# LucasAlegre/morl-baselines

Measured on NVIDIA B200. Metric: envelope_q_updates_per_sec, higher is better.
Workload: dtype f32

## Files before the change

### include/morl_b200.h

```cpp
#ifndef MORL_B200_H_
#define MORL_B200_H_

#include <stddef.h>
#include <stdint.h>

#ifdef __cplusplus
extern "C" {
#endif

#define MORL_B200_VERSION 100

#if defined(__GNUC__)
#define MORL_API __attribute__((visibility("default")))
#else
#define MORL_API
#endif

#define MORL_OK 0
#define MORL_ERR_NULL (-1)
#define MORL_ERR_SHAPE (-2)
#define MORL_ERR_ALIGN (-3)
#define MORL_ERR_UNSUPPORTED (-4)
#define MORL_ERR_NO_DEVICE (-5)

// ... 116 lines not shown
                                 float* q_out, void* stream);
MORL_API int morl_qhead_envelope_td_f32(int fmt, const void* a_on_planes, const void* a_tg_planes, long long a_plane_stride,
                                        const float* a_scale_on, const float* a_scale_tg, const void* w_on_planes, const void* w_tg_planes,
                                        long long w_plane_stride, const float* w_scale_on, const float* w_scale_tg, const float* bias_on,
                                        const float* bias_tg, int K, const float* wset, const float* reward, const float* done, float gamma,
                                        int B, int W, int A, int D, int dot_mode, int row_order, int reverse_tiles, float* target_out,
                                        int32_t* pref_out, int32_t* act_out, float* q_on_out, float* q_tg_out, void* stream);
MORL_API int morl_pairs_relu_split_planes(int fmt, const float* u, const float* v, int B, int W, int H, void* dst_planes,
                                          long long plane_stride, const float* scale, void* relu_bits_out, void* stream);


MORL_API size_t morl_gemm_mn_workspace_bytes(int M, int a_cols, int b_cols);
MORL_API int morl_gemm_planes_mn_f32(int fmt, const void* g_planes, long long g_plane_stride, int ldg, int g_cols, const float* g_scale,
                                     const void* h_planes, long long h_plane_stride, int ldh, int h_cols, const float* h_scale, int M,
                                     int transpose_out, float* out, int ld_out, float* colsum_out, void* workspace, void* stream);
MORL_API int morl_colsum_planes(int fmt, const void* planes, long long plane_stride, const float* scale, int M, int ld, int N, float* out,
                                void* workspace, void* stream);
MORL_API int morl_pairs_grad_reduce_planes(int fmt, const void* planes, long long plane_stride, const float* scale, int B, int W, int H,
                                           float* dU, float* dV, void* workspace, void* stream);

MORL_API int morl_pair_layer1_uv_f32(const float* feats, const float* wset, const float* W1, const float* b1, int B, int W, int F, int D, int H,
                                     float* u, float* v, void* stream);

MORL_API size_t morl_pair_layer1_grad_workspace_bytes(int F, int D, int H);
MORL_API int morl_pair_layer1_grad_f32(const float* dU, const float* dV, const float* feats, const float* wset, int B, int W, int F,
                              int D, int H, float* dW1, float* db1, void* workspace, void* stream);


MORL_API size_t morl_adam_workspace_bytes(int n_tensors, int64_t max_size);
MORL_API int morl_adam_clip_f32(float* const* params, const float* const* grads, float* const* exp_avg, float* const* exp_avg_sq,
// ... 8 lines not shown
```

### morl_baselines_b200/_lib.py

```python

from __future__ import annotations

import ctypes as C
import os

HERE = os.path.dirname(os.path.abspath(__file__))
LIB_PATH = os.path.join(HERE, "csrc", "libmorl_b200.so")

DOT_UNFUSED, DOT_FMA, DOT_PAIRFMA = 0, 1, 2
MAP_TILE, MAP_BLOCK = 0, 1
ROWS_REFERENCE, ROWS_BMAJOR = 0, 1
AC_ELEMENTWISE_MIN, AC_SCALAR_MIN, AC_ARGMIN_GATHER = 0, 1, 2
MAX_D = 8
FMT_BF16X3, FMT_F16X2 = 0, 1

_vp, _i, _f, _d, _i64, _sz = C.c_void_p, C.c_int, C.c_float, C.c_double, C.c_int64, C.c_size_t

SIGNATURES = {
    "morl_version": (_i, []),
    "morl_last_error": (C.c_char_p, []),
    "morl_device_sm_count": (_i, []),
    "morl_envelope_td_f32": (_i, [_vp, _vp, _vp, _vp, _vp, _f, _i, _i, _i, _i, _i, _i, _vp, _vp, _vp, _vp]),
    "morl_greedy_td_f32": (_i, [_vp, _vp, _vp, _i, _i, _vp, _vp, _i, _i, _f, _i, _i, _i, _i, _vp, _vp, _vp]),
    "morl_critic_min_td_f32": (_i, [_vp, _i, _vp, _i, _i, _vp, _vp, _i, _i, _f, _i, _i, _i, _i, _vp, _vp, _vp]),
# ... 23 lines not shown
    "morl_split_planes": (_i, [_i, _vp, _i, _i, _i, _i, _vp, _i, _i, C.c_longlong, _vp, _vp]),
    "morl_gemm_planes_f32": (_i, [_i, _vp, C.c_longlong, _vp, _vp, C.c_longlong, _vp, _i, _i, _i, _i, _vp, _i, _vp, _i, _vp, _i, _vp, _i, C.c_longlong,
                                  _vp, _i, _i, _vp, _vp, _vp]),
    "morl_gemm_chain_supported": (_i, [_i, _i, _i]),
    "morl_gemm_chain_f32": (_i, [_i, _i, _i, _vp, C.c_longlong, _vp, _vp, C.c_longlong, _vp, _vp, _i, _vp, _vp, _i, _i, _i, _vp]),
    "morl_debug_gemm_stats": (_i, [_vp, _i]),
    "morl_ensemble_sample_f32": (_i, [_vp, _vp, _vp, _vp, _vp, _vp, _i, _i, _i, _i, _vp, _vp, _vp, _vp]),
    "morl_qhead_envelope_supported": (_i, [_i, _i, _i, _i, _i, _i]),
    "morl_qhead_gemm_supported": (_i, [_i, _i, _i, _i]),
    "morl_qhead_gemm_f32": (_i, [_i, _vp, C.c_longlong, _vp, _vp, C.c_longlong, _vp, _vp, _i, _i, _i, _i, _vp, _vp]),
    "morl_qhead_envelope_td_f32": (_i, [_i, _vp, _vp, C.c_longlong, _vp, _vp, _vp, _vp, C.c_longlong, _vp, _vp, _vp, _vp, _i, _vp, _vp, _vp, _f, _i, _i,
                                        _i, _i, _i, _i, _i, _vp, _vp, _vp, _vp, _vp, _vp]),
    "morl_pairs_relu_split_planes": (_i, [_i, _vp, _vp, _i, _i, _i, _vp, C.c_longlong, _vp, _vp, _vp]),
    "morl_gemm_mn_workspace_bytes": (_sz, [_i, _i, _i]),
    "morl_gemm_planes_mn_f32": (_i, [_i, _vp, C.c_longlong, _i, _i, _vp, _vp, C.c_longlong, _i, _i, _vp, _i, _i, _vp, _i, _vp, _vp, _vp]),
    "morl_colsum_planes": (_i, [_i, _vp, C.c_longlong, _vp, _i, _i, _i, _vp, _vp, _vp]),
    "morl_pairs_grad_reduce_planes": (_i, [_i, _vp, C.c_longlong, _vp, _i, _i, _i, _vp, _vp, _vp, _vp]),
    "morl_pair_layer1_uv_f32": (_i, [_vp, _vp, _vp, _vp, _i, _i, _i, _i, _i, _vp, _vp, _vp]),
    "morl_pair_layer1_grad_workspace_bytes": (_sz, [_i, _i, _i]),
    "morl_pair_layer1_grad_f32": (_i, [_vp, _vp, _vp, _vp, _i, _i, _i, _i, _i, _vp, _vp, _vp, _vp]),
    "morl_adam_workspace_bytes": (_sz, [_i, _i64]),
    "morl_adam_clip_f32": (_i, [_vp, _vp, _vp, _vp, _vp, _vp, _i, _i64, _f, _f, _f, _f, _f, _vp, _vp]),
}

SPLIT_MAX_JOBS = 16


class SplitJob(C.Structure):

    _fields_ = [("src", _vp), ("dst_planes", _vp), ("plane_stride", C.c_longlong), ("scale", _vp), ("rows", _i), ("cols", _i), ("ld_src", _i),
                ("transpose", _i), ("rows_pad", _i), ("ldp", _i), ("auto_scale", _i), ("target_exp", _i)]


_lib = None


class MorlB200Error(RuntimeError):
    pass


def load():
    global _lib
    if _lib is not None:
        return _lib
    if not os.path.exists(LIB_PATH):
        raise MorlB200Error(
# ... 17 lines not shown
```

### morl_baselines_b200/csrc/gemm_planes.cu

```cuda
#include <cuda.h>
#include <cuda_bf16.h>
#include <cuda_fp16.h>
#include <stdlib.h>
#include <string.h>

#include "common.cuh"
#include "gemm_tc.cuh"

namespace morl {

constexpr int kGemmBM = 128;
constexpr int kGemmThreads = 320;

__device__ unsigned int g_plane_overflow;


__device__ __forceinline__ void note_overflow(float amax) {
    if (amax > 65504.f) atomicAdd(&g_plane_overflow, 1u);
}

#define MORL_DISPATCH_FMT(F_, ...)                                                         \
    switch (F_) {                                                                          \
        case MORL_FMT_BF16X3: { constexpr int kFmt = MORL_FMT_BF16X3; __VA_ARGS__; } break; \
        case MORL_FMT_F16X2: { constexpr int kFmt = MORL_FMT_F16X2; __VA_ARGS__; } break;   \
// ... 842 lines not shown
            uint32_t v[32];
            tc_ld32(t_row + 256u, v);
            tc_ld_wait();
            g.colsum_partial[(size_t)split * g.n_tiles * 128 + row] = n_kblk > 0 ? __uint_as_float(v[0]) : 0.f;
        }
    }
    tc_fence_before();
    __syncthreads();
    if (MC) cluster_sync_all();
    if (warp == 1) {
        tc_fence_after();
        asm volatile("tcgen05.dealloc.cta_group::1.sync.aligned.b32 %0, 512;" ::"r"(tmem_base) : "memory");
    }
}

__global__ void __launch_bounds__(256) reduce_partials_kernel(const float* __restrict__ partial, int S, int prow, int pcol, int rows, int cols,
                                                              int transpose, float* __restrict__ out, int ld_out, int main_blocks,
                                                              const float* __restrict__ vec_partial, float* __restrict__ vec_out,
                                                              const float* __restrict__ scale_a, const float* __restrict__ scale_b) {
    pdl_enter();
    __shared__ float red[8][33];
    float mul = 1.0f / (ld_scale(scale_a) * ld_scale(scale_b));
    if ((int)blockIdx.x >= main_blocks) {
        partial = vec_partial;
        out = vec_out;
        pcol = 1; cols = 1; transpose = 0; ld_out = 1;
        mul = 1.0f / ld_scale(scale_a);
    }
    const int e = ((int)blockIdx.x >= main_blocks ? (int)blockIdx.x - main_blocks : (int)blockIdx.x) * 32 + threadIdx.x;
    const int total = rows * cols;
// ... 15 lines not shown
    }
    red[threadIdx.y][threadIdx.x] = acc;
    __syncthreads();
    if (threadIdx.y == 0 && e < total) {
        float t = red[0][threadIdx.x];
#pragma unroll
        for (int y = 1; y < 8; ++y) t += red[y][threadIdx.x];
        t *= mul;
        if (transpose)
            out[(size_t)c * ld_out + r] = t;
        else
            out[(size_t)r * ld_out + c] = t;
    }
}

__global__ void __launch_bounds__(256) reduce_partials_vec4_kernel(const float* __restrict__ partial, int S, int prow, int pcol, int rows, int cols,
                                                                   float* __restrict__ out, int ld_out, int main_blocks,
                                                                   const float* __restrict__ vec_partial, float* __restrict__ vec_out,
                                                                   const float* __restrict__ scale_a, const float* __restrict__ scale_b) {
    pdl_enter();
    __shared__ float4 red[8][33];
    if ((int)blockIdx.x >= main_blocks) {
        const float mul = 1.0f / ld_scale(scale_a);
        const int e = ((int)blockIdx.x - main_blocks) * 32 + threadIdx.x;
        float acc = 0.f;
        if (e < rows) {
            const float* p = vec_partial + e;
            float a0 = 0.f, a1 = 0.f;
            int s = threadIdx.y;
            for (; s + 8 < S; s += 16) {
                a0 += p[(size_t)s * prow];
                a1 += p[(size_t)(s + 8) * prow];
            }
            if (s < S) a0 += p[(size_t)s * prow];
            acc = a0 + a1;
        }
        red[threadIdx.y][threadIdx.x].x = acc;
        __syncthreads();
        if (threadIdx.y == 0 && e < rows) {
            float t = red[0][threadIdx.x].x;
#pragma unroll
            for (int y = 1; y < 8; ++y) t += red[y][threadIdx.x].x;
            vec_out[e] = t * mul;
        }
        return;
    }
    const float mul = 1.0f / (ld_scale(scale_a) * ld_scale(scale_b));
    const int e4 = ((int)blockIdx.x * 32 + threadIdx.x) * 4;
    const int total = rows * cols;
    float4 acc = make_float4(0.f, 0.f, 0.f, 0.f);
    int r = 0, c = 0;
    if (e4 < total) {
        r = e4 / cols;
        c = e4 - r * cols;
        const float* p = partial + (size_t)r * pcol + c;
        const size_t stride = (size_t)prow * pcol;
        constexpr int kRedMax = 12;
        float4 a0 = acc, a1 = acc;
        if (S <= 8 * kRedMax) {
            float4 v[kRedMax];
#pragma unroll
            for (int k = 0; k < kRedMax; ++k) {
                const int sk = threadIdx.y + 8 * k;
// ... 20 lines not shown
            }
        }
        acc = make_float4(a0.x + a1.x, a0.y + a1.y, a0.z + a1.z, a0.w + a1.w);
    }
    red[threadIdx.y][threadIdx.x] = acc;
    __syncthreads();
    if (threadIdx.y == 0 && e4 < total) {
        float4 t = red[0][threadIdx.x];
#pragma unroll
        for (int y = 1; y < 8; ++y) {
            const float4 q = red[y][threadIdx.x];
            t.x += q.x; t.y += q.y; t.z += q.z; t.w += q.w;
        }
        *reinterpret_cast<float4*>(out + (size_t)r * ld_out + c) = make_float4(t.x * mul, t.y * mul, t.z * mul, t.w * mul);
    }
}

template <int FMT>
__global__ void __launch_bounds__(256) colsum_planes_kernel(const uint16_t* __restrict__ planes, long long plane_stride, int M, int ld, int N,
                                                            int rows_per_chunk, float* __restrict__ part) {
    using F = PlaneFmt<FMT>;
    __shared__ float red[8][32][9];
    const int n0 = (blockIdx.y * 32 + threadIdx.x) * 8;
    const int m0 = blockIdx.x * rows_per_chunk, m1 = min(M, m0 + rows_per_chunk);
    float acc[8];
#pragma unroll
    for (int j = 0; j < 8; ++j) acc[j] = 0.f;
    if (n0 < ld) {
        for (int m = m0 + threadIdx.y; m < m1; m += 8) {
            const size_t o = (size_t)m * ld + n0;
// ... 384 lines not shown
static int make_plane_map_mn(CUtensorMap* map, int fmt, const void* base, int rows, int ld, long long plane_stride_elems) {
    EncodeTiledFn enc = get_encode_fn();
    if (!enc) return -1;
    const cuuint32_t P = (cuuint32_t)fmt_planes(fmt);
    const cuuint64_t dims[3] = {(cuuint64_t)ld, (cuuint64_t)rows, P};
    const cuuint64_t strides[2] = {(cuuint64_t)ld * 2, (cuuint64_t)plane_stride_elems * 2};
    const cuuint32_t box[3] = {64, (cuuint32_t)kMnKT, P};
    const cuuint32_t estr[3] = {1, 1, 1};
    const CUresult r = enc(map, fmt_tm_type(fmt), 3, const_cast<void*>(base), dims, strides, box, estr, CU_TENSOR_MAP_INTERLEAVE_NONE,
                           CU_TENSOR_MAP_SWIZZLE_128B, CU_TENSOR_MAP_L2_PROMOTION_L2_128B, CU_TENSOR_MAP_FLOAT_OOB_FILL_NONE);
    return r == CUDA_SUCCESS ? 0 : (int)r;
}

static inline bool fmt_ok(int fmt) { return fmt == MORL_FMT_BF16X3 || fmt == MORL_FMT_F16X2; }

}

extern "C" int morl_plane_overflow_count(int reset) {
    using namespace morl;
    unsigned int v = 0;
    cudaDeviceSynchronize();
    if (cudaMemcpyFromSymbol(&v, g_plane_overflow, sizeof(v)) != cudaSuccess) {
        (void)cudaGetLastError();
        set_error("morl_plane_overflow_count: no CUDA device");
        return MORL_ERR_NO_DEVICE;
    }
    if (reset) {
        const unsigned int z = 0;
        cudaMemcpyToSymbol(g_plane_overflow, &z, sizeof(z));
    }
// ... 2 lines not shown

extern "C" int morl_amax_scale_f32(const float* src, long long n, int target_exp, float* scale_out, void* workspace, void* stream) {
    using namespace morl;
    MORL_REQUIRE(src && scale_out && workspace, MORL_ERR_NULL, "morl_amax_scale_f32: NULL pointer argument");
    MORL_REQUIRE(n > 0 && target_exp >= -14 && target_exp <= 15, MORL_ERR_SHAPE, "morl_amax_scale_f32: bad n=%lld / target_exp=%d", n, target_exp);
    long long blocks = (n / 4 + 255) / 256;
    if (blocks > 148) blocks = 148;
    if (blocks < 1) blocks = 1;
    launch_k(amax_scale_kernel, dim3((int)blocks), dim3(256), 0, static_cast<cudaStream_t>(stream), src, n, target_exp, scale_out, static_cast<unsigned int*>(workspace));
    return check_launch("morl_amax_scale_f32");
}

extern "C" size_t morl_gemm_mn_workspace_bytes(int M, int a_cols, int b_cols) {
    if (M <= 0 || a_cols <= 0 || b_cols <= 0) return 0;
    const int n_tiles = (a_cols + 127) / 128;
    int S = 148 / n_tiles;
    if (S < 1) S = 1;
    int rps = ((M + S - 1) / S + 31) / 32 * 32;
    S = (M + rps - 1) / rps;
    const int NB = (b_cols + 63) / 64 * 64;
    return (size_t)S * n_tiles * 128 * NB * sizeof(float) + (size_t)256 * 256 * sizeof(float);
}

extern "C" int morl_gemm_planes_mn_f32(int fmt, const void* g_planes, long long g_plane_stride, int ldg, int g_cols, const float* g_scale,
                                       const void* h_planes, long long h_plane_stride, int ldh, int h_cols, const float* h_scale, int M,
                                       int transpose_out, float* out, int ld_out, float* colsum_out, void* workspace, void* stream) {
    using namespace morl;
    MORL_REQUIRE(fmt_ok(fmt), MORL_ERR_UNSUPPORTED, "morl_gemm_planes_mn_f32: unknown plane format %d", fmt);
    MORL_REQUIRE(g_planes && h_planes && out && workspace, MORL_ERR_NULL, "morl_gemm_planes_mn_f32: NULL pointer argument");
    MORL_REQUIRE(M > 0 && g_cols > 0 && h_cols > 0, MORL_ERR_SHAPE, "morl_gemm_planes_mn_f32: bad shape M=%d g_cols=%d h_cols=%d", M, g_cols, h_cols);
    MORL_REQUIRE(ldg % 64 == 0 && ldh % 64 == 0 && ldh <= 256 && g_cols <= ldg && h_cols <= ldh, MORL_ERR_UNSUPPORTED,
                 "morl_gemm_planes_mn_f32: plane row lengths must be multiples of 64 (ldg=%d ldh=%d), ldh <= 256", ldg, ldh);
    const int n_tiles = (g_cols + 127) / 128;
    MORL_REQUIRE(n_tiles * 128 <= ldg || ldg % 128 == 0 || n_tiles * 128 - ldg <= 64, MORL_ERR_UNSUPPORTED, "morl_gemm_planes_mn_f32: ldg=%d", ldg);
    int S = 148 / n_tiles;
    if (S < 1) S = 1;
    const int rps = ((M + S - 1) / S + 31) / 32 * 32;
    S = (M + rps - 1) / rps;
    const int NB = (h_cols + 63) / 64 * 64;
    CUtensorMap tmA, tmB;
    int rc = make_plane_map_mn(&tmA, fmt, g_planes, M, ldg, g_plane_stride);
    MORL_REQUIRE(rc == 0, MORL_ERR_NO_DEVICE, "morl_gemm_planes_mn_f32: cuTensorMapEncodeTiled(G) failed (%d)", rc);
    rc = make_plane_map_mn(&tmB, fmt, h_planes, M, ldh, h_plane_stride);
    MORL_REQUIRE(rc == 0, MORL_ERR_NO_DEVICE, "morl_gemm_planes_mn_f32: cuTensorMapEncodeTiled(H) failed (%d)", rc);
    GemmMnArgs g;
    g.M = M; g.n_tiles = n_tiles; g.NB = NB; g.rows_per_split = rps; g.partial = static_cast<float*>(workspace);
    g.colsum_partial = colsum_out ? g.partial + (size_t)S * n_tiles * 128 * NB : nullptr;
    cudaStream_t st = static_cast<cudaStream_t>(stream);
    MORL_DISPATCH_FMT(fmt, {
        using F = PlaneFmt<kFmt>;
        const size_t smem = (size_t)F::kStagesMn * (6u * F::P * kMnKT * 128u) + 256 + 1024 + 64 + 1024 + 4096;
        static bool attr_set = false, attr_set_mc = false;
        if (!attr_set) {
            cudaFuncSetAttribute(gemm_planes_mn_kernel<kFmt, 0>, cudaFuncAttributeMaxDynamicSharedMemorySize, (int)smem);
            attr_set = true;
        }
        static const bool mc_env = [] { const char* e = getenv("MORL_MN_MULTICAST"); return e && e[0] == '1'; }();
        if (mc_env && n_tiles == 2 && NB == 256) {
            if (!attr_set_mc) {
                cudaFuncSetAttribute(gemm_planes_mn_kernel<kFmt, 1>, cudaFuncAttributeMaxDynamicSharedMemorySize, (int)smem);
                attr_set_mc = true;
            }
            cudaLaunchConfig_t cfg;
            memset(&cfg, 0, sizeof(cfg));
            cfg.gridDim = dim3(n_tiles * S);
            cfg.blockDim = dim3(192);
// ... 14 lines not shown
        }
    });
    rc = check_launch("morl_gemm_planes_mn_f32");
    if (rc) return rc;
    const int total = g_cols * h_cols;
    const int main_blocks = (total + 31) / 32, vec_blocks = colsum_out ? (g_cols + 31) / 32 : 0;
    if (!transpose_out && h_cols % 4 == 0 && ld_out % 4 == 0 && aligned16(out)) {
        const int mb4 = (total / 4 + 31) / 32;
        launch_k(reduce_partials_vec4_kernel, dim3(mb4 + vec_blocks), dim3(dim3(32, 8)), 0, st, g.partial, S, n_tiles * 128, NB, g_cols, h_cols, out, ld_out, mb4,
                                                                              g.colsum_partial, colsum_out, g_scale, h_scale);
        return check_launch("morl_gemm_planes_mn_f32(reduce)");
    }
    launch_k(reduce_partials_kernel, dim3(main_blocks + vec_blocks), dim3(dim3(32, 8)), 0, st, g.partial, S, n_tiles * 128, NB, g_cols, h_cols, transpose_out, out, ld_out,
                                                                             main_blocks, g.colsum_partial, colsum_out, g_scale, h_scale);
    return check_launch("morl_gemm_planes_mn_f32(reduce)");
}

extern "C" int morl_colsum_planes(int fmt, const void* planes, long long plane_stride, const float* scale, int M, int ld, int N, float* out,
                                  void* workspace, void* stream) {
    using namespace morl;
    MORL_REQUIRE(fmt_ok(fmt), MORL_ERR_UNSUPPORTED, "morl_colsum_planes: unknown plane format %d", fmt);
    MORL_REQUIRE(planes && out && workspace, MORL_ERR_NULL, "morl_colsum_planes: NULL pointer argument");
    MORL_REQUIRE(M > 0 && N > 0 && ld >= N && ld % 8 == 0 && plane_stride % 8 == 0, MORL_ERR_SHAPE, "morl_colsum_planes: bad shape M=%d N=%d ld=%d", M, N, ld);
    const int chunks = 296;
    const int rpc = (M + chunks - 1) / chunks;
    const int nch = (M + rpc - 1) / rpc;
    cudaStream_t st = static_cast<cudaStream_t>(stream);
    float* part = static_cast<float*>(workspace);
    MORL_DISPATCH_FMT(fmt, (colsum_planes_kernel<kFmt><<<dim3((unsigned)nch, (unsigned)((ld + 255) / 256)), dim3(32, 8), 0, st>>>(
                               static_cast<const uint16_t*>(planes), plane_stride, M, ld, N, rpc, part)));
// ... 367 lines not shown
```

### morl_baselines_b200/csrc/gemm_tc.cuh

```cuda
#pragma once
#include <cuda.h>
#include <cuda_bf16.h>
#include <cuda_fp16.h>

#include "common.cuh"

namespace morl {

__device__ __forceinline__ uint32_t g_smem_u32(const void* p) { return (uint32_t)__cvta_generic_to_shared(p); }

__device__ __forceinline__ void g_mbar_init(uint64_t* bar, int count) {
    asm volatile("mbarrier.init.shared::cta.b64 [%0], %1;" ::"r"(g_smem_u32(bar)), "r"(count));
}
__device__ __forceinline__ void g_mbar_expect_tx(uint64_t* bar, uint32_t bytes) {
    asm volatile("mbarrier.arrive.expect_tx.shared::cta.b64 _, [%0], %1;" ::"r"(g_smem_u32(bar)), "r"(bytes) : "memory");
}
__device__ __forceinline__ void g_mbar_arrive(uint64_t* bar) {
    asm volatile("mbarrier.arrive.shared::cta.b64 _, [%0];" ::"r"(g_smem_u32(bar)) : "memory");
}
__device__ __forceinline__ void g_mbar_wait(uint64_t* bar, uint32_t parity) {
    uint32_t ok = 0;
    for (uint32_t it = 0; it < (1u << 26); ++it) {
        asm volatile(
            "{\n\t.reg .pred p;\n\t"
// ... 87 lines not shown
        "{\n\t.reg .pred p;\n\t"
        "setp.ne.b32 p, %4, 0;\n\t"
        "tcgen05.mma.cta_group::1.kind::f16 [%0], %1, %2, %3, p;\n\t}" ::"r"(tmem_d),
        "l"(adesc), "l"(bdesc), "r"(idesc), "r"(accumulate)
        : "memory");
}
__device__ __forceinline__ void tc_ld32(uint32_t taddr, uint32_t (&v)[32]) {
    asm volatile(
        "tcgen05.ld.sync.aligned.32x32b.x32.b32 {%0, %1, %2, %3, %4, %5, %6, %7, %8, %9, %10, %11, %12, %13, %14, %15, %16, %17, %18, %19, "
        "%20, %21, %22, %23, %24, %25, %26, %27, %28, %29, %30, %31}, [%32];"
        : "=r"(v[0]), "=r"(v[1]), "=r"(v[2]), "=r"(v[3]), "=r"(v[4]), "=r"(v[5]), "=r"(v[6]), "=r"(v[7]), "=r"(v[8]), "=r"(v[9]), "=r"(v[10]),
          "=r"(v[11]), "=r"(v[12]), "=r"(v[13]), "=r"(v[14]), "=r"(v[15]), "=r"(v[16]), "=r"(v[17]), "=r"(v[18]), "=r"(v[19]), "=r"(v[20]),
          "=r"(v[21]), "=r"(v[22]), "=r"(v[23]), "=r"(v[24]), "=r"(v[25]), "=r"(v[26]), "=r"(v[27]), "=r"(v[28]), "=r"(v[29]), "=r"(v[30]),
          "=r"(v[31])
        : "r"(taddr));
}
__device__ __forceinline__ void tc_ld_wait() { asm volatile("tcgen05.wait::ld.sync.aligned;" ::: "memory"); }

template <int FMT>
struct PlaneFmt;

template <>
struct PlaneFmt<MORL_FMT_BF16X3> {
    static constexpr int P = 3, NPROD = 6;
    static constexpr int BK = 32;
    static constexpr uint32_t kIdescAB = (1u << 7) | (1u << 10);
    static constexpr uint32_t kOnes2 = 0x3F803F80u;
    static constexpr int kStages1 = 2, kStages2 = 3, kStagesMn = 3;
    __device__ static constexpr int pa(int t) { return t == 0 ? 2 : (t == 2 || t == 3) ? 1 : 0; }
    __device__ static constexpr int pb(int t) { return t == 1 ? 2 : (t == 2 || t == 4) ? 1 : 0; }
// ... 110 lines not shown
```

### morl_baselines_b200/ops.py

```python

from __future__ import annotations

from typing import Optional, Tuple

import torch as th

from . import _lib
from ._lib import (
    AC_ARGMIN_GATHER,
    AC_ELEMENTWISE_MIN,
    AC_SCALAR_MIN,
    DOT_FMA,
    DOT_PAIRFMA,
    DOT_UNFUSED,
    MAP_BLOCK,
    MAP_TILE,
    ROWS_BMAJOR,
    ROWS_REFERENCE,
)

launch_count = 0


def _count(n=1):
# ... 572 lines not shown
    _, M, ldg = g_planes.shape
    _, M2, ldh = h_planes.shape
    if M != M2 or fmt_of(h_planes) != fmt:
        raise _lib.MorlB200Error("gemm_planes_mn: plane tensors must share format and number of rows")
    dev = g_planes.device
    if out is None:
        out = th.empty((h_cols, g_cols) if transpose_out else (g_cols, h_cols), device=dev, dtype=th.float32)
    ws = gemm_mn_workspace(M, g_cols, h_cols, dev) if workspace is None else workspace
    rc = _lib.load().morl_gemm_planes_mn_f32(fmt, _ptr(g_planes), g_planes.stride(0), ldg, g_cols, _ptr(g_scale), _ptr(h_planes), h_planes.stride(0), ldh,
                                             h_cols, _ptr(h_scale), M, int(transpose_out), _ptr(out), out.stride(0), _ptr(colsum), _ptr(ws), _stream())
    _lib.check(rc, "morl_gemm_planes_mn_f32")
    _count(2)
    return out


def colsum_planes(planes: th.Tensor, n_cols: int, out: Optional[th.Tensor] = None, workspace: Optional[th.Tensor] = None,
                  scale: Optional[th.Tensor] = None) -> th.Tensor:
    fmt = fmt_of(planes)
    _, M, ld = planes.shape
    dev = planes.device
    out = th.empty(n_cols, device=dev, dtype=th.float32) if out is None else out
    ws = th.empty(296 * n_cols, device=dev, dtype=th.float32) if workspace is None else workspace
    rc = _lib.load().morl_colsum_planes(fmt, _ptr(planes), planes.stride(0), _ptr(scale), M, ld, n_cols, _ptr(out), _ptr(ws), _stream())
    _lib.check(rc, "morl_colsum_planes")
    _count(2)
    return out


def pairs_grad_reduce(planes: th.Tensor, B: int, W: int, workspace: Optional[th.Tensor] = None, dU: Optional[th.Tensor] = None,
                      dV: Optional[th.Tensor] = None, scale: Optional[th.Tensor] = None):
# ... 11 lines not shown
```

### morl_baselines_b200/tc_mlp.py

```python

from __future__ import annotations

import os
from typing import List, Optional

import torch as th
from torch import nn

from . import ops

_SNAKE = os.environ.get("MORL_TC_SNAKE", "1") == "1"
_CHAIN = os.environ.get("MORL_GEMM_CHAIN", "1") == "1"
_CHAIN_BWD = os.environ.get("MORL_GEMM_CHAIN_BWD", "1") == "1"
_NARROW_HEAD = os.environ.get("MORL_NARROW_HEAD", "1") == "1"
_DEFAULT_FMT = ops.FMT_BF16X3 if os.environ.get("MORL_TC_FMT", "f16x2") == "bf16x3" else ops.FMT_F16X2

ACT_SCALE = 2.0
W_TARGET_EXP = 14
G_TARGET_EXP = 2


def _pad(n: int, m: int) -> int:
    return (n + m - 1) // m * m


class TCPairMlp:

    @staticmethod
# ... 27 lines not shown
            raise ops._lib.MorlB200Error("TCPairMlp: unsupported network (Linear/ReLU stack with hidden widths that are multiples of 64 (f16x2) or "
                                         "32 (bf16x3) and <= 256)")
        dev = self.lin[0].weight.device
        M = n_obs * n_w
        scaled = fmt == ops.FMT_F16X2
        self.h = [ops.empty_planes(fmt, M, l.out_features, dev) for l in self.lin[:-1]]
        self.s_act = ops.scale_tensor(ACT_SCALE, dev) if scaled else None
        if share_weights_with is not None:
            if share_weights_with.fmt != fmt:
                raise ops._lib.MorlB200Error("TCPairMlp: plans sharing weight planes must use the same operand format")
            self.wp, self.s_w = share_weights_with.wp, share_weights_with.s_w
        else:
            self.wp = [ops.empty_planes(fmt, _pad(l.out_features, 32), l.in_features, dev) for l in self.lin[1:]]
            self.s_w = [ops.scale_tensor(1.0, dev) if scaled else None for _ in self.lin[1:]]
        self.q = th.empty((M, self.lin[-1].out_features), device=dev, dtype=th.float32)
        self._chain = self._gchain = self._gbufs = None
        self.trainable = trainable
        if trainable:
            if n_w > 64:
                raise ops._lib.MorlB200Error("TCPairMlp backward supports at most 64 weight vectors per minibatch")
            out = self.lin[-1].out_features
            self.ld_last = _pad(out, 64)
            hid = max(l.out_features for l in self.lin[:-1])
            self.g_last = ops.empty_planes(fmt, M, self.ld_last, dev)
            self.g = [ops.empty_planes(fmt, M, hid, dev) for _ in range(2)]
            self.hbits = [ops.empty_relu_bits(M, dev) for _ in self.lin[:-1]]
            self.s_g = ops.scale_tensor(1.0, dev) if scaled else None
            self.ws_amax = th.zeros(2, device=dev, dtype=th.int32)
            self.wtp = []
            for k, l in enumerate(self.lin[1:], start=1):
                kdim = self.ld_last if k == len(self.lin) - 1 else l.out_features
# ... 129 lines not shown
            after_gemms()
        dU, dV = ops.pairs_grad_reduce(G, self.B, self.W, workspace=self.ws_red, dU=self.dU, dV=self.dV, scale=self.s_g)
        grads[0], grads[1] = ops.pair_layer1_grad(dU, dV, feats, wset, dW1=grads[0], db1=grads[1], workspace=self.ws_l1)
        return grads


def _backward_chained(self, feats, wset, G, grads, after_gemms):
    n = len(self.lin)
    dev = G.device
    if self._gchain is None:
        M, hid = self.B * self.W, self.lin[1].in_features
        self._gbufs = [ops.empty_planes(self.fmt, M, hid, dev) for _ in range(n - 1)]
        ks = list(range(n - 1, 0, -1))
        self._gchain = ops.GemmChain([[self.g_last] + self._gbufs], [[self.wtp[k - 1] for k in ks]], None, [[self.s_w[k - 1] for k in ks]], None,
                                     act_scale=self.s_g, relu=False, bits_in=[[self.hbits[k - 1] for k in ks]], k_first=self.ld_last)
    last = self.lin[n - 1]
    if grads[2 * (n - 1) + 1] is None:
        grads[2 * (n - 1) + 1] = th.empty(last.out_features, device=dev, dtype=th.float32)
    grads[2 * (n - 1)] = ops.gemm_planes_mn(G, last.out_features, self.h[n - 2], last.in_features, out=grads[2 * (n - 1)], workspace=self.ws_mn,
                                            colsum=grads[2 * (n - 1) + 1], g_scale=self.s_g, h_scale=self.s_act)
    self._gchain()
    for i, k in enumerate(range(n - 2, 0, -1)):
        l = self.lin[k]
        if grads[2 * k + 1] is None:
            grads[2 * k + 1] = th.empty(l.out_features, device=dev, dtype=th.float32)
        grads[2 * k] = ops.gemm_planes_mn(self._gbufs[i], l.out_features, self.h[k - 1], l.in_features, out=grads[2 * k], workspace=self.ws_mn,
                                          colsum=grads[2 * k + 1], g_scale=self.s_g, h_scale=self.s_act)
    if after_gemms is not None:
        after_gemms()
    dU, dV = ops.pairs_grad_reduce(self._gbufs[n - 2], self.B, self.W, workspace=self.ws_red, dU=self.dU, dV=self.dV, scale=self.s_g)
    grads[0], grads[1] = ops.pair_layer1_grad(dU, dV, feats, wset, dW1=grads[0], db1=grads[1], workspace=self.ws_l1)
    return grads


TCPairMlp._backward_chained = _backward_chained


class TCPairMlpFn(th.autograd.Function):

    @staticmethod
    def forward(ctx, plan: TCPairMlp, feats: th.Tensor, wset: th.Tensor, *params):
        q = plan.forward_pairs(feats, wset)
        ctx.plan = plan
        ctx.save_for_backward(feats, wset)
        return q

    @staticmethod
    def backward(ctx, dq):
        feats, wset = ctx.saved_tensors
        grads = ctx.plan.backward(feats, wset, dq.contiguous())
# ... 2 lines not shown
```

Baseline: 1563.

## Batch all backward weight-gradient GEMMs into one multi-job tcgen05 launch

Adds a multi-job MN GEMM kernel that computes every layer's weight gradient and bias column-sum in one persistent launch, followed by one shared split-K reduction launch. Previously each layer issued its own GEMM and reduce kernels, serialised after the gradient chain. This cuts launch count and lets small per-layer products share the SMs. The cost is a new job-lookup path in the kernel, a cached descriptor set keyed on gradient pointers, and the last-layer GEMM now waits until after the chain instead of overlapping with it.

```diff
diff --git a/include/morl_b200.h b/include/morl_b200.h
--- a/include/morl_b200.h
+++ b/include/morl_b200.h
@@ -154,6 +154,20 @@
 MORL_API int morl_gemm_planes_mn_f32(int fmt, const void* g_planes, long long g_plane_stride, int ldg, int g_cols, const float* g_scale,
                                      const void* h_planes, long long h_plane_stride, int ldh, int h_cols, const float* h_scale, int M,
                                      int transpose_out, float* out, int ld_out, float* colsum_out, void* workspace, void* stream);
+#define MORL_MN_MAX_JOBS 4
+typedef struct MorlMnJob {
+    const void* g_planes;
+    long long g_plane_stride;
+    const float* g_scale;
+    const void* h_planes;
+    long long h_plane_stride;
+    const float* h_scale;
+    float* out;
+    float* colsum_out;
+    int ldg, g_cols, ldh, h_cols, ld_out;
+} MorlMnJob;
+MORL_API size_t morl_gemm_mn_multi_workspace_bytes(const MorlMnJob* jobs, int n_jobs, int M);
+MORL_API int morl_gemm_planes_mn_multi_f32(int fmt, const MorlMnJob* jobs, int n_jobs, int M, void* workspace, void* stream);
 MORL_API int morl_colsum_planes(int fmt, const void* planes, long long plane_stride, const float* scale, int M, int ld, int N, float* out,
                                 void* workspace, void* stream);
 MORL_API int morl_pairs_grad_reduce_planes(int fmt, const void* planes, long long plane_stride, const float* scale, int B, int W, int H,
diff --git a/morl_baselines_b200/_lib.py b/morl_baselines_b200/_lib.py
--- a/morl_baselines_b200/_lib.py
+++ b/morl_baselines_b200/_lib.py
@@ -61,6 +61,8 @@
     "morl_pairs_relu_split_planes": (_i, [_i, _vp, _vp, _i, _i, _i, _vp, C.c_longlong, _vp, _vp, _vp]),
     "morl_gemm_mn_workspace_bytes": (_sz, [_i, _i, _i]),
     "morl_gemm_planes_mn_f32": (_i, [_i, _vp, C.c_longlong, _i, _i, _vp, _vp, C.c_longlong, _i, _i, _vp, _i, _i, _vp, _i, _vp, _vp, _vp]),
+    "morl_gemm_mn_multi_workspace_bytes": (_sz, [_vp, _i, _i]),
+    "morl_gemm_planes_mn_multi_f32": (_i, [_i, _vp, _i, _i, _vp, _vp]),
     "morl_colsum_planes": (_i, [_i, _vp, C.c_longlong, _vp, _i, _i, _i, _vp, _vp, _vp]),
     "morl_pairs_grad_reduce_planes": (_i, [_i, _vp, C.c_longlong, _vp, _i, _i, _i, _vp, _vp, _vp, _vp]),
     "morl_pair_layer1_uv_f32": (_i, [_vp, _vp, _vp, _vp, _i, _i, _i, _i, _i, _vp, _vp, _vp]),
@@ -77,6 +79,15 @@
 
     _fields_ = [("src", _vp), ("dst_planes", _vp), ("plane_stride", C.c_longlong), ("scale", _vp), ("rows", _i), ("cols", _i), ("ld_src", _i),
                 ("transpose", _i), ("rows_pad", _i), ("ldp", _i), ("auto_scale", _i), ("target_exp", _i)]
+
+
+MN_MAX_JOBS = 4
+
+
+class MnJob(C.Structure):
+
+    _fields_ = [("g_planes", _vp), ("g_plane_stride", C.c_longlong), ("g_scale", _vp), ("h_planes", _vp), ("h_plane_stride", C.c_longlong),
+                ("h_scale", _vp), ("out", _vp), ("colsum_out", _vp), ("ldg", _i), ("g_cols", _i), ("ldh", _i), ("h_cols", _i), ("ld_out", _i)]
 
 
 _lib = None
diff --git a/morl_baselines_b200/csrc/gemm_planes.cu b/morl_baselines_b200/csrc/gemm_planes.cu
--- a/morl_baselines_b200/csrc/gemm_planes.cu
+++ b/morl_baselines_b200/csrc/gemm_planes.cu
@@ -880,6 +880,204 @@
     }
 }
 
+template <int FMT>
+constexpr size_t mn_smem_bytes() {
+    return (size_t)PlaneFmt<FMT>::kStagesMn * (6u * PlaneFmt<FMT>::P * kMnKT * 128u) + 256 + 1024 + 64 + 1024 + 4096;
+}
+
+constexpr int kMnMaxJobs = MORL_MN_MAX_JOBS;
+
+struct MnJobArgs {
+    int n_tiles, NB, rows_per_split, S;
+    int g_cols, h_cols, ld_out;
+    int unit0;
+    int red_block0, red_main_blocks;
+    float* partial;
+    float* colsum_partial;
+    float* out;
+    float* colsum_out;
+    const float* g_scale;
+    const float* h_scale;
+};
+
+struct alignas(64) MnMulti {
+    CUtensorMap tmA[kMnMaxJobs], tmB[kMnMaxJobs];
+    MnJobArgs job[kMnMaxJobs];
+    int n_jobs, n_units, M;
+};
+
+template <int FMT>
+__global__ void __launch_bounds__(kGemmThreads, 1) gemm_planes_mn_multi_kernel(const __grid_constant__ MnMulti mj) {
+    using F = PlaneFmt<FMT>;
+    constexpr int P = F::P;
+    constexpr int kStages = F::kStagesMn;
+    extern __shared__ uint8_t gsmem_raw[];
+    uint8_t* gsmem = gsmem_raw + ((1024u - (g_smem_u32(gsmem_raw) & 1023u)) & 1023u);
+    constexpr uint32_t chunk_bytes = (uint32_t)P * kMnKT * 128u;
+    constexpr uint32_t a_stage = 2u * chunk_bytes;
+    constexpr uint32_t b_stage = 4u * chunk_bytes;
+    uint8_t* smA = gsmem;
+    uint8_t* smB = gsmem + kStages * a_stage;
+    uint64_t* full = reinterpret_cast<uint64_t*>(smB + kStages * b_stage);
+    uint64_t* empty = full + kStages;
+    uint64_t* tfull = empty + kStages;
+    uint64_t* tempty = tfull + 1;
+    uint32_t* tmem_slot = reinterpret_cast<uint32_t*>(tempty + 1);
+    uint8_t* ones_b = reinterpret_cast<uint8_t*>(tmem_slot + 4);
+    uint32_t* ones = reinterpret_cast<uint32_t*>(ones_b + ((1024u - (g_smem_u32(ones_b) & 1023u)) & 1023u));
+    for (int t = threadIdx.x; t < 1024; t += blockDim.x) ones[t] = F::kOnes2;
+    asm volatile("fence.proxy.async.shared::cta;" ::: "memory");
+
+    const int warp = threadIdx.x >> 5, lane = threadIdx.x & 31;
+    auto job_of = [&](int u) {
+        int j = 0;
+        while (j + 1 < mj.n_jobs && u >= mj.job[j + 1].unit0) ++j;
+        return j;
+    };
+    auto unit_of = [&](int u, int& j, int& nt, int& split, int& m_begin, int& n_kblk) {
+        j = job_of(u);
+        const MnJobArgs& jb = mj.job[j];
+        const int l = u - jb.unit0;
+        nt = l % jb.n_tiles;
+        split = l / jb.n_tiles;
+        m_begin = split * jb.rows_per_split;
+        const int m_end = min(mj.M, m_begin + jb.rows_per_split);
+        n_kblk = (m_end - m_begin + kMnKT - 1) / kMnKT;
+    };
+
+    if (threadIdx.x == 0) {
+        for (int s = 0; s < kStages; ++s) {
+            g_mbar_init(&full[s], 1);
+            g_mbar_init(&empty[s], 1);
+        }
+        g_mbar_init(tfull, 1);
+        g_mbar_init(tempty, 8);
+        asm volatile("fence.mbarrier_init.release.cluster;" ::: "memory");
+    }
+    if (warp == 1) {
+        asm volatile("tcgen05.alloc.cta_group::1.sync.aligned.shared::cta.b32 [%0], 512;" ::"r"(g_smem_u32(tmem_slot)) : "memory");
+        asm volatile("tcgen05.relinquish_alloc_permit.cta_group::1.sync.aligned;" ::: "memory");
+    }
+    tc_fence_before();
+    __syncthreads();
+    tc_fence_after();
+    const uint32_t tmem_base = *tmem_slot;
+    pdl_enter();
+
+    if (warp == 0) {
+        if (lane == 0) {
+            uint32_t stage = 0, phase = 0;
+            for (int u = blockIdx.x; u < mj.n_units; u += gridDim.x) {
+                int j, nt, split, m_begin, n_kblk;
+                unit_of(u, j, nt, split, m_begin, n_kblk);
+                const CUtensorMap* tmA = &mj.tmA[j];
+                const CUtensorMap* tmB = &mj.tmB[j];
+                const int nb_chunks = mj.job[j].NB / 64;
+                for (int kb = 0; kb < n_kblk; ++kb) {
+                    g_mbar_wait(&empty[stage], phase ^ 1u);
+                    g_mbar_expect_tx(&full[stage], (2u + (uint32_t)nb_chunks) * chunk_bytes);
+                    const int m0 = m_begin + kb * kMnKT;
+                    for (int c = 0; c < 2; ++c) tma_load_3d(smA + stage * a_stage + c * chunk_bytes, tmA, &full[stage], nt * 128 + c * 64, m0, 0);
+                    for (int c = 0; c < nb_chunks; ++c) tma_load_3d(smB + stage * b_stage + c * chunk_bytes, tmB, &full[stage], c * 64, m0, 0);
+                    if (++stage == kStages) {
+                        stage = 0;
+                        phase ^= 1u;
+                    }
+                }
+            }
+        }
+    } else if (warp == 1) {
+        if (lane == 0) {
+            const uint32_t idesc_ones = (1u << 4) | F::kIdescAB | (1u << 15) | (1u << 16) | ((uint32_t)(16 >> 3) << 17) | ((uint32_t)(128 >> 4) << 24);
+            const uint64_t ones_desc = make_desc_mn_sw128(g_smem_u32(ones), chunk_bytes);
+            constexpr uint32_t plane = kMnKT * 128u;
+            uint32_t stage = 0, phase = 0, it = 0;
+            for (int u = blockIdx.x; u < mj.n_units; u += gridDim.x, ++it) {
+                int j, nt, split, m_begin, n_kblk;
+                unit_of(u, j, nt, split, m_begin, n_kblk);
+                const bool colsum = mj.job[j].colsum_partial != nullptr;
+                const uint32_t idesc = (1u << 4) | F::kIdescAB | (1u << 15) | (1u << 16) | ((uint32_t)(mj.job[j].NB >> 3) << 17) | ((uint32_t)(128 >> 4) << 24);
+                g_mbar_wait(tempty, (it & 1u) ^ 1u);
+                tc_fence_after();
+                for (int kb = 0; kb < n_kblk; ++kb) {
+                    g_mbar_wait(&full[stage], phase);
+                    tc_fence_after();
+                    const uint32_t a0 = g_smem_u32(smA + stage * a_stage);
+                    const uint32_t b0 = g_smem_u32(smB + stage * b_stage);
+#pragma unroll
+                    for (int ks = 0; ks < kMnKT / 16; ++ks) {
+#pragma unroll
+                        for (int t = 0; t < F::NPROD; ++t) {
+                            const uint64_t ad = make_desc_mn_sw128(a0 + F::pa(t) * plane + ks * 2048u, chunk_bytes);
+                            const uint64_t bd = make_desc_mn_sw128(b0 + F::pb(t) * plane + ks * 2048u, chunk_bytes);
+                            tc_mma_bf16(tmem_base, ad, bd, idesc, (kb | ks | t) != 0 ? 1u : 0u);
+                        }
+                        if (colsum) {
+#pragma unroll
+                            for (int pl = P - 1; pl >= 0; --pl)
+                                tc_mma_bf16(tmem_base + 256u, make_desc_mn_sw128(a0 + pl * plane + ks * 2048u, chunk_bytes), ones_desc, idesc_ones,
+                                            (kb | ks | (P - 1 - pl)) != 0 ? 1u : 0u);
+                        }
+                    }
+                    tc_commit(&empty[stage]);
+                    if (++stage == kStages) {
+                        stage = 0;
+                        phase ^= 1u;
+                    }
+                }
+                tc_commit(tfull);
+            }
+        }
+    } else {
+        const int quad = warp & 3;
+        const int half = (warp - 2) >> 2;
+        const uint32_t t_row = tmem_base + ((uint32_t)(quad * 32) << 16);
+        uint32_t it = 0;
+        for (int u = blockIdx.x; u < mj.n_units; u += gridDim.x, ++it) {
+            const int j = job_of(u);
+            const int ncol = mj.job[j].NB >> 1;
+            const bool colsum = half == 0 && mj.job[j].colsum_partial != nullptr;
+            g_mbar_wait(tfull, it & 1u);
+            tc_fence_after();
+            uint32_t cs = 0;
+            if (colsum) cs = tc_ld1(t_row + 256u);
+            uint32_t v[4][32];
+#pragma unroll
+            for (int c = 0; c < 4; ++c)
+                if (c * 32 < ncol) tc_ld32(t_row + (uint32_t)(half * ncol + c * 32), v[c]);
+            tc_ld_wait();
+#pragma unroll
+            for (int c = 0; c < 4; ++c)
+#pragma unroll
+                for (int e = 0; e < 32; ++e) asm volatile("" : "+r"(v[c][e]));
+            tc_fence_before();
+            __syncwarp();
+            if (lane == 0) g_mbar_arrive(tempty);
+            const MnJobArgs& jb = mj.job[j];
+            const int l = u - jb.unit0, nt = l % jb.n_tiles, split = l / jb.n_tiles;
+            const int row = nt * 128 + quad * 32 + lane;
+            if (row < jb.g_cols) {
+                float* prow = jb.partial + ((size_t)split * jb.g_cols + row) * jb.NB + half * ncol;
+#pragma unroll
+                for (int c = 0; c < 4; ++c)
+                    if (c * 32 < ncol) {
+#pragma unroll
+                        for (int e = 0; e < 32; e += 4)
+                            *reinterpret_cast<float4*>(prow + c * 32 + e) = make_float4(__uint_as_float(v[c][e]), __uint_as_float(v[c][e + 1]),
+                                                                                         __uint_as_float(v[c][e + 2]), __uint_as_float(v[c][e + 3]));
+                    }
+                if (colsum) jb.colsum_partial[(size_t)split * jb.g_cols + row] = __uint_as_float(cs);
+            }
+        }
+    }
+    tc_fence_before();
+    __syncthreads();
+    if (warp == 1) {
+        tc_fence_after();
+        asm volatile("tcgen05.dealloc.cta_group::1.sync.aligned.b32 %0, 512;" ::"r"(tmem_base) : "memory");
+    }
+}
+
 __global__ void __launch_bounds__(256) reduce_partials_kernel(const float* __restrict__ partial, int S, int prow, int pcol, int rows, int cols,
                                                               int transpose, float* __restrict__ out, int ld_out, int main_blocks,
                                                               const float* __restrict__ vec_partial, float* __restrict__ vec_out,
@@ -925,15 +1123,13 @@
     }
 }
 
-__global__ void __launch_bounds__(256) reduce_partials_vec4_kernel(const float* __restrict__ partial, int S, int prow, int pcol, int rows, int cols,
-                                                                   float* __restrict__ out, int ld_out, int main_blocks,
-                                                                   const float* __restrict__ vec_partial, float* __restrict__ vec_out,
-                                                                   const float* __restrict__ scale_a, const float* __restrict__ scale_b) {
-    pdl_enter();
+__device__ __forceinline__ void reduce_partials_vec4_block(int block, const float* __restrict__ partial, int S, int prow, int pcol, int rows, int cols,
+                                                           float* __restrict__ out, int ld_out, int main_blocks, const float* __restrict__ vec_partial,
+                                                           float* __restrict__ vec_out, const float* __restrict__ scale_a, const float* __restrict__ scale_b) {
     __shared__ float4 red[8][33];
-    if ((int)blockIdx.x >= main_blocks) {
+    if (block >= main_blocks) {
         const float mul = 1.0f / ld_scale(scale_a);
-        const int e = ((int)blockIdx.x - main_blocks) * 32 + threadIdx.x;
+        const int e = (block - main_blocks) * 32 + threadIdx.x;
         float acc = 0.f;
         if (e < rows) {
             const float* p = vec_partial + e;
@@ -957,7 +1153,7 @@
         return;
     }
     const float mul = 1.0f / (ld_scale(scale_a) * ld_scale(scale_b));
-    const int e4 = ((int)blockIdx.x * 32 + threadIdx.x) * 4;
+    const int e4 = (block * 32 + threadIdx.x) * 4;
     const int total = rows * cols;
     float4 acc = make_float4(0.f, 0.f, 0.f, 0.f);
     int r = 0, c = 0;
@@ -1008,6 +1204,23 @@
         }
         *reinterpret_cast<float4*>(out + (size_t)r * ld_out + c) = make_float4(t.x * mul, t.y * mul, t.z * mul, t.w * mul);
     }
+}
+
+__global__ void __launch_bounds__(256) reduce_partials_vec4_kernel(const float* __restrict__ partial, int S, int prow, int pcol, int rows, int cols,
+                                                                   float* __restrict__ out, int ld_out, int main_blocks,
+                                                                   const float* __restrict__ vec_partial, float* __restrict__ vec_out,
+                                                                   const float* __restrict__ scale_a, const float* __restrict__ scale_b) {
+    pdl_enter();
+    reduce_partials_vec4_block((int)blockIdx.x, partial, S, prow, pcol, rows, cols, out, ld_out, main_blocks, vec_partial, vec_out, scale_a, scale_b);
+}
+
+__global__ void __launch_bounds__(256) reduce_partials_vec4_multi_kernel(const __grid_constant__ MnMulti mj) {
+    pdl_enter();
+    int j = 0;
+    while (j + 1 < mj.n_jobs && (int)blockIdx.x >= mj.job[j + 1].red_block0) ++j;
+    const MnJobArgs& jb = mj.job[j];
+    reduce_partials_vec4_block((int)blockIdx.x - jb.red_block0, jb.partial, jb.S, jb.g_cols, jb.NB, jb.g_cols, jb.h_cols, jb.out, jb.ld_out, jb.red_main_blocks,
+                               jb.colsum_partial, jb.colsum_out, jb.g_scale, jb.h_scale);
 }
 
 template <int FMT>
@@ -1422,6 +1635,20 @@
 
 static inline bool fmt_ok(int fmt) { return fmt == MORL_FMT_BF16X3 || fmt == MORL_FMT_F16X2; }
 
+static inline void mn_split(int M, int n_tiles, int& S, int& rps) {
+    S = 148 / n_tiles;
+    if (S < 1) S = 1;
+    rps = ((M + S - 1) / S + kMnKT - 1) / kMnKT * kMnKT;
+    S = (M + rps - 1) / rps;
+}
+
+static inline size_t mn_multi_job_floats(int M, int g_cols, int h_cols) {
+    int S, rps;
+    mn_split(M, (g_cols + 127) / 128, S, rps);
+    const size_t nb = (size_t)((h_cols + 63) / 64 * 64);
+    return (size_t)S * g_cols * nb + ((size_t)S * g_cols + 3) / 4 * 4;
+}
+
 }
 
 extern "C" int morl_plane_overflow_count(int reset) {
@@ -1454,10 +1681,8 @@
 extern "C" size_t morl_gemm_mn_workspace_bytes(int M, int a_cols, int b_cols) {
     if (M <= 0 || a_cols <= 0 || b_cols <= 0) return 0;
     const int n_tiles = (a_cols + 127) / 128;
-    int S = 148 / n_tiles;
-    if (S < 1) S = 1;
-    int rps = ((M + S - 1) / S + 31) / 32 * 32;
-    S = (M + rps - 1) / rps;
+    int S, rps;
+    morl::mn_split(M, n_tiles, S, rps);
     const int NB = (b_cols + 63) / 64 * 64;
     return (size_t)S * n_tiles * 128 * NB * sizeof(float) + (size_t)256 * 256 * sizeof(float);
 }
@@ -1473,10 +1698,8 @@
                  "morl_gemm_planes_mn_f32: plane row lengths must be multiples of 64 (ldg=%d ldh=%d), ldh <= 256", ldg, ldh);
     const int n_tiles = (g_cols + 127) / 128;
     MORL_REQUIRE(n_tiles * 128 <= ldg || ldg % 128 == 0 || n_tiles * 128 - ldg <= 64, MORL_ERR_UNSUPPORTED, "morl_gemm_planes_mn_f32: ldg=%d", ldg);
-    int S = 148 / n_tiles;
-    if (S < 1) S = 1;
-    const int rps = ((M + S - 1) / S + 31) / 32 * 32;
-    S = (M + rps - 1) / rps;
+    int S, rps;
+    mn_split(M, n_tiles, S, rps);
     const int NB = (h_cols + 63) / 64 * 64;
     CUtensorMap tmA, tmB;
     int rc = make_plane_map_mn(&tmA, fmt, g_planes, M, ldg, g_plane_stride);
@@ -1488,8 +1711,7 @@
     g.colsum_partial = colsum_out ? g.partial + (size_t)S * n_tiles * 128 * NB : nullptr;
     cudaStream_t st = static_cast<cudaStream_t>(stream);
     MORL_DISPATCH_FMT(fmt, {
-        using F = PlaneFmt<kFmt>;
-        const size_t smem = (size_t)F::kStagesMn * (6u * F::P * kMnKT * 128u) + 256 + 1024 + 64 + 1024 + 4096;
+        const size_t smem = mn_smem_bytes<kFmt>();
         static bool attr_set = false, attr_set_mc = false;
         if (!attr_set) {
             cudaFuncSetAttribute(gemm_planes_mn_kernel<kFmt, 0>, cudaFuncAttributeMaxDynamicSharedMemorySize, (int)smem);
@@ -1534,6 +1756,80 @@
     launch_k(reduce_partials_kernel, dim3(main_blocks + vec_blocks), dim3(dim3(32, 8)), 0, st, g.partial, S, n_tiles * 128, NB, g_cols, h_cols, transpose_out, out, ld_out,
                                                                              main_blocks, g.colsum_partial, colsum_out, g_scale, h_scale);
     return check_launch("morl_gemm_planes_mn_f32(reduce)");
+}
+
+extern "C" size_t morl_gemm_mn_multi_workspace_bytes(const MorlMnJob* jobs, int n_jobs, int M) {
+    using namespace morl;
+    if (!jobs || n_jobs <= 0 || n_jobs > kMnMaxJobs || M <= 0) return 0;
+    size_t floats = 0;
+    for (int i = 0; i < n_jobs; ++i) {
+        if (jobs[i].g_cols <= 0 || jobs[i].h_cols <= 0) return 0;
+        floats += mn_multi_job_floats(M, jobs[i].g_cols, jobs[i].h_cols);
+    }
+    return floats * sizeof(float);
+}
+
+extern "C" int morl_gemm_planes_mn_multi_f32(int fmt, const MorlMnJob* jobs, int n_jobs, int M, void* workspace, void* stream) {
+    using namespace morl;
+    MORL_REQUIRE(fmt_ok(fmt), MORL_ERR_UNSUPPORTED, "morl_gemm_planes_mn_multi_f32: unknown plane format %d", fmt);
+    MORL_REQUIRE(jobs && workspace, MORL_ERR_NULL, "morl_gemm_planes_mn_multi_f32: NULL pointer argument");
+    MORL_REQUIRE(n_jobs >= 1 && n_jobs <= kMnMaxJobs && M > 0, MORL_ERR_SHAPE, "morl_gemm_planes_mn_multi_f32: bad n_jobs=%d / M=%d (1 <= n_jobs <= %d)", n_jobs, M,
+                 kMnMaxJobs);
+    MORL_REQUIRE(aligned16(workspace), MORL_ERR_ALIGN, "morl_gemm_planes_mn_multi_f32: workspace must be 16-byte aligned");
+    MnMulti mj;
+    memset(&mj, 0, sizeof(mj));
+    mj.n_jobs = n_jobs;
+    mj.M = M;
+    float* ws = static_cast<float*>(workspace);
+    int units = 0, red_blocks = 0;
+    for (int i = 0; i < n_jobs; ++i) {
+        const MorlMnJob& q = jobs[i];
+        MORL_REQUIRE(q.g_planes && q.h_planes && q.out, MORL_ERR_NULL, "morl_gemm_planes_mn_multi_f32: job %d has a NULL pointer", i);
+        MORL_REQUIRE(q.g_cols > 0 && q.h_cols > 0 && q.ldg % 64 == 0 && q.ldh % 64 == 0 && q.ldh <= 256 && q.g_cols <= q.ldg && q.h_cols <= q.ldh,
+                     MORL_ERR_SHAPE, "morl_gemm_planes_mn_multi_f32: job %d: bad shape g_cols=%d ldg=%d h_cols=%d ldh=%d (ld multiples of 64, ldh <= 256)", i,
+                     q.g_cols, q.ldg, q.h_cols, q.ldh);
+        const int n_tiles = (q.g_cols + 127) / 128;
+        MORL_REQUIRE(n_tiles * 128 <= q.ldg || q.ldg % 128 == 0 || n_tiles * 128 - q.ldg <= 64, MORL_ERR_UNSUPPORTED,
+                     "morl_gemm_planes_mn_multi_f32: job %d: ldg=%d", i, q.ldg);
+        MORL_REQUIRE(q.h_cols % 4 == 0 && q.ld_out >= q.h_cols && q.ld_out % 4 == 0 && aligned16(q.out), MORL_ERR_UNSUPPORTED,
+                     "morl_gemm_planes_mn_multi_f32: job %d: needs h_cols %% 4 == 0, ld_out %% 4 == 0 (>= h_cols) and a 16-byte aligned output", i);
+        MnJobArgs& a = mj.job[i];
+        mn_split(M, n_tiles, a.S, a.rows_per_split);
+        a.n_tiles = n_tiles;
+        a.NB = (q.h_cols + 63) / 64 * 64;
+        a.g_cols = q.g_cols; a.h_cols = q.h_cols; a.ld_out = q.ld_out;
+        a.unit0 = units;
+        units += n_tiles * a.S;
+        a.partial = ws;
+        a.colsum_partial = q.colsum_out ? ws + (size_t)a.S * q.g_cols * a.NB : nullptr;
+        ws += mn_multi_job_floats(M, q.g_cols, q.h_cols);
+        a.out = q.out; a.colsum_out = q.colsum_out; a.g_scale = q.g_scale; a.h_scale = q.h_scale;
+        a.red_block0 = red_blocks;
+        a.red_main_blocks = (q.g_cols * q.h_cols / 4 + 31) / 32;
+        red_blocks += a.red_main_blocks + (q.colsum_out ? (q.g_cols + 31) / 32 : 0);
+        int rc = make_plane_map_mn(&mj.tmA[i], fmt, q.g_planes, M, q.ldg, q.g_plane_stride);
+        MORL_REQUIRE(rc == 0, MORL_ERR_NO_DEVICE, "morl_gemm_planes_mn_multi_f32: job %d: cuTensorMapEncodeTiled(G) failed (%d)", i, rc);
+        rc = make_plane_map_mn(&mj.tmB[i], fmt, q.h_planes, M, q.ldh, q.h_plane_stride);
+        MORL_REQUIRE(rc == 0, MORL_ERR_NO_DEVICE, "morl_gemm_planes_mn_multi_f32: job %d: cuTensorMapEncodeTiled(H) failed (%d)", i, rc);
+    }
+    mj.n_units = units;
+    int sms = morl_device_sm_count();
+    if (sms <= 0) sms = 148;
+    const int grid = units < sms ? units : sms;
+    cudaStream_t st = static_cast<cudaStream_t>(stream);
+    MORL_DISPATCH_FMT(fmt, {
+        constexpr size_t smem = mn_smem_bytes<kFmt>();
+        static bool attr_set = false;
+        if (!attr_set) {
+            cudaFuncSetAttribute(gemm_planes_mn_multi_kernel<kFmt>, cudaFuncAttributeMaxDynamicSharedMemorySize, (int)smem);
+            attr_set = true;
+        }
+        launch_k(gemm_planes_mn_multi_kernel<kFmt>, dim3(grid), dim3(kGemmThreads), smem, st, mj);
+    });
+    const int rc = check_launch("morl_gemm_planes_mn_multi_f32");
+    if (rc) return rc;
+    launch_k(reduce_partials_vec4_multi_kernel, dim3(red_blocks), dim3(32, 8), 0, st, mj);
+    return check_launch("morl_gemm_planes_mn_multi_f32(reduce)");
 }
 
 extern "C" int morl_colsum_planes(int fmt, const void* planes, long long plane_stride, const float* scale, int M, int ld, int N, float* out,
diff --git a/morl_baselines_b200/csrc/gemm_tc.cuh b/morl_baselines_b200/csrc/gemm_tc.cuh
--- a/morl_baselines_b200/csrc/gemm_tc.cuh
+++ b/morl_baselines_b200/csrc/gemm_tc.cuh
@@ -125,6 +125,11 @@
           "=r"(v[21]), "=r"(v[22]), "=r"(v[23]), "=r"(v[24]), "=r"(v[25]), "=r"(v[26]), "=r"(v[27]), "=r"(v[28]), "=r"(v[29]), "=r"(v[30]),
           "=r"(v[31])
         : "r"(taddr));
+}
+__device__ __forceinline__ uint32_t tc_ld1(uint32_t taddr) {
+    uint32_t v;
+    asm volatile("tcgen05.ld.sync.aligned.32x32b.x1.b32 {%0}, [%1];\n\ttcgen05.wait::ld.sync.aligned;" : "=r"(v) : "r"(taddr) : "memory");
+    return v;
 }
 __device__ __forceinline__ void tc_ld_wait() { asm volatile("tcgen05.wait::ld.sync.aligned;" ::: "memory"); }
 
diff --git a/morl_baselines_b200/ops.py b/morl_baselines_b200/ops.py
--- a/morl_baselines_b200/ops.py
+++ b/morl_baselines_b200/ops.py
@@ -610,6 +610,36 @@
     return out
 
 
+class GemmMnMulti:
+
+    def __init__(self, jobs):
+        if not 1 <= len(jobs) <= _lib.MN_MAX_JOBS:
+            raise _lib.MorlB200Error(f"GemmMnMulti: 1 to {_lib.MN_MAX_JOBS} products per launch (got {len(jobs)})")
+        self.fmt = fmt_of(jobs[0][0])
+        self.M = jobs[0][0].shape[1]
+        arr = (_lib.MnJob * len(jobs))()
+        for i, (g, gc, h, hc, out, colsum, sg, sh) in enumerate(jobs):
+            if fmt_of(g) != self.fmt or fmt_of(h) != self.fmt or g.shape[1] != self.M or h.shape[1] != self.M:
+                raise _lib.MorlB200Error("GemmMnMulti: plane tensors must share format and number of rows")
+            if tuple(out.shape) != (gc, hc) or out.stride(1) != 1 or out.dtype != th.float32:
+                raise _lib.MorlB200Error(f"GemmMnMulti: job {i}: out must be fp32 [{gc}, {hc}] with unit column stride")
+            if colsum is not None and (colsum.numel() < gc or colsum.dtype != th.float32 or not colsum.is_contiguous()):
+                raise _lib.MorlB200Error(f"GemmMnMulti: job {i}: colsum must be a contiguous fp32 tensor of {gc} elements")
+            arr[i] = _lib.MnJob(_ptr(g), g.stride(0), _ptr(sg), _ptr(h), h.stride(0), _ptr(sh), _ptr(out), _ptr(colsum), g.shape[2], int(gc), h.shape[2],
+                                int(hc), out.stride(0))
+        self._jobs, self._n = arr, len(jobs)
+        self._keep = jobs
+        nbytes = _lib.load().morl_gemm_mn_multi_workspace_bytes(arr, self._n, self.M)
+        if nbytes == 0:
+            raise _lib.MorlB200Error("GemmMnMulti: bad job shapes")
+        self.workspace = th.empty((nbytes + 3) // 4, device=jobs[0][0].device, dtype=th.float32)
+
+    def __call__(self):
+        rc = _lib.load().morl_gemm_planes_mn_multi_f32(self.fmt, self._jobs, self._n, self.M, _ptr(self.workspace), _stream())
+        _lib.check(rc, "morl_gemm_planes_mn_multi_f32")
+        _count(2)
+
+
 def colsum_planes(planes: th.Tensor, n_cols: int, out: Optional[th.Tensor] = None, workspace: Optional[th.Tensor] = None,
                   scale: Optional[th.Tensor] = None) -> th.Tensor:
     fmt = fmt_of(planes)
diff --git a/morl_baselines_b200/tc_mlp.py b/morl_baselines_b200/tc_mlp.py
--- a/morl_baselines_b200/tc_mlp.py
+++ b/morl_baselines_b200/tc_mlp.py
@@ -12,6 +12,7 @@
 _SNAKE = os.environ.get("MORL_TC_SNAKE", "1") == "1"
 _CHAIN = os.environ.get("MORL_GEMM_CHAIN", "1") == "1"
 _CHAIN_BWD = os.environ.get("MORL_GEMM_CHAIN_BWD", "1") == "1"
+_MN_MULTI = os.environ.get("MORL_MN_MULTI", "1") == "1"
 _NARROW_HEAD = os.environ.get("MORL_NARROW_HEAD", "1") == "1"
 _DEFAULT_FMT = ops.FMT_BF16X3 if os.environ.get("MORL_TC_FMT", "f16x2") == "bf16x3" else ops.FMT_F16X2
 
@@ -69,7 +70,7 @@
             self.wp = [ops.empty_planes(fmt, _pad(l.out_features, 32), l.in_features, dev) for l in self.lin[1:]]
             self.s_w = [ops.scale_tensor(1.0, dev) if scaled else None for _ in self.lin[1:]]
         self.q = th.empty((M, self.lin[-1].out_features), device=dev, dtype=th.float32)
-        self._chain = self._gchain = self._gbufs = None
+        self._chain = self._gchain = self._gbufs = self._mn_multi = None
         self.trainable = trainable
         if trainable:
             if n_w > 64:
@@ -229,26 +230,43 @@
         ks = list(range(n - 1, 0, -1))
         self._gchain = ops.GemmChain([[self.g_last] + self._gbufs], [[self.wtp[k - 1] for k in ks]], None, [[self.s_w[k - 1] for k in ks]], None,
                                      act_scale=self.s_g, relu=False, bits_in=[[self.hbits[k - 1] for k in ks]], k_first=self.ld_last)
+    for k in range(1, n):
+        if grads[2 * k] is None:
+            grads[2 * k] = th.empty((self.lin[k].out_features, self.lin[k].in_features), device=dev, dtype=th.float32)
+        if grads[2 * k + 1] is None:
+            grads[2 * k + 1] = th.empty(self.lin[k].out_features, device=dev, dtype=th.float32)
+    if _MN_MULTI and n - 1 <= ops._lib.MN_MAX_JOBS:
+        self._gchain()
+        key = tuple(grads[i].data_ptr() for i in range(2, 2 * n))
+        if self._mn_multi is None or self._mn_multi[0] != key:
+            jobs = [(self._gbufs[n - 2 - k], self.lin[k].out_features, self.h[k - 1], self.lin[k].in_features, grads[2 * k], grads[2 * k + 1], self.s_g,
+                     self.s_act) for k in range(1, n - 1)]
+            jobs.append((G, self.lin[n - 1].out_features, self.h[n - 2], self.lin[n - 1].in_features, grads[2 * (n - 1)], grads[2 * (n - 1) + 1], self.s_g,
+                         self.s_act))
+            self._mn_multi = (key, ops.GemmMnMulti(jobs))
+        self._mn_multi[1]()
+        return self._backward_tail(feats, wset, grads, after_gemms)
     last = self.lin[n - 1]
-    if grads[2 * (n - 1) + 1] is None:
-        grads[2 * (n - 1) + 1] = th.empty(last.out_features, device=dev, dtype=th.float32)
     grads[2 * (n - 1)] = ops.gemm_planes_mn(G, last.out_features, self.h[n - 2], last.in_features, out=grads[2 * (n - 1)], workspace=self.ws_mn,
                                             colsum=grads[2 * (n - 1) + 1], g_scale=self.s_g, h_scale=self.s_act)
     self._gchain()
     for i, k in enumerate(range(n - 2, 0, -1)):
         l = self.lin[k]
-        if grads[2 * k + 1] is None:
-            grads[2 * k + 1] = th.empty(l.out_features, device=dev, dtype=th.float32)
         grads[2 * k] = ops.gemm_planes_mn(self._gbufs[i], l.out_features, self.h[k - 1], l.in_features, out=grads[2 * k], workspace=self.ws_mn,
                                           colsum=grads[2 * k + 1], g_scale=self.s_g, h_scale=self.s_act)
+    return self._backward_tail(feats, wset, grads, after_gemms)
+
+
+def _backward_tail(self, feats, wset, grads, after_gemms):
     if after_gemms is not None:
         after_gemms()
-    dU, dV = ops.pairs_grad_reduce(self._gbufs[n - 2], self.B, self.W, workspace=self.ws_red, dU=self.dU, dV=self.dV, scale=self.s_g)
+    dU, dV = ops.pairs_grad_reduce(self._gbufs[len(self.lin) - 2], self.B, self.W, workspace=self.ws_red, dU=self.dU, dV=self.dV, scale=self.s_g)
     grads[0], grads[1] = ops.pair_layer1_grad(dU, dV, feats, wset, dW1=grads[0], db1=grads[1], workspace=self.ws_l1)
     return grads
 
 
 TCPairMlp._backward_chained = _backward_chained
+TCPairMlp._backward_tail = _backward_tail
 
 
 class TCPairMlpFn(th.autograd.Function):
```

Result: faster. 1647, median of 6 (+5.4%).
